# mct10/Speech-Vecalign

Measured on AMD Instinct MI355X. Metric: aligned doc-pairs/sec, higher is better.
Workload: dtype bf16; 1 GPU; synthetic 4096x4096 d=1024 bf16 embeddings, 4 overlap layers/side, 10 alignment types, band 14, coarse-to-fine (max_size_full_dp=300), 1024 doc-pairs per GPU per step; pipeline=1, N=4096, M=4096, d=1024, overlaps=4, parallelism=dp1 (pairs sharded, no collective)

## Files before the change

include/svx.h:

```cpp
#ifndef SVX_H
#define SVX_H

#include <stdint.h>

#ifdef __cplusplus
extern "C" {
#endif

typedef struct svx_ctx svx_ctx;

enum svx_dtype { SVX_F32 = 0, SVX_F16 = 1, SVX_BF16 = 2 };

enum svx_status {
    SVX_OK = 0,
    SVX_ERR_ARG = 1,
    SVX_ERR_OVERLAPS = 2,
    SVX_ERR_HIP = 3,
    SVX_ERR_TRACEBACK = 4,
    SVX_ERR_NOMEM = 5,
    SVX_ERR_EXTEND = 6,
    SVX_ERR_PATH = 7,
    SVX_ERR_BP = 8
};

// ... 150 lines not shown

typedef struct svx_level_view {
    int32_t size0, size1, k0, k1;
    int32_t n_types, band;
    int32_t path_len, n_align;
    const float *n0, *n1;
    const double *del_penalty;
    const int32_t *searchpath;
    const float *a_b_costs;
    const int32_t *b_offset;
    const double *a_b_csum;
    const uint8_t *a_b_bp;
    const int32_t *a_b_xp, *a_b_yp;
    const int32_t *new_b_offset;
    const int32_t *alignments;
    const double *alignment_scores;
    const float *costs_1to1;
    const int32_t *x_y_tb_diag;
    const float *v0_l0, *v1_l0;
    const float *knob_scores;
    int32_t n_knob, reserved;
} svx_level_view;
int svx_debug_level(svx_ctx *ctx, int pair, int level, svx_level_view *out);
int svx_copy_to_host(svx_ctx *ctx, void *dst_host, const void *src_device, int64_t bytes);

int svx_set_profiling(svx_ctx *ctx, int on);
int svx_set_pipeline(svx_ctx *ctx, int on);
int svx_flush(svx_ctx *ctx);
double svx_stage_ms(svx_ctx *ctx, const char *stage);
int svx_stage_launches(svx_ctx *ctx, const char *stage);

#ifdef __cplusplus
}
#endif
#endif
```

speech-vecalign_amd/csrc/svx_api.hip:

```cpp
#include <stdarg.h>
#include <stdio.h>
#include <stdlib.h>
#include <string.h>

#include <chrono>
#include <functional>
#include <memory>
#include <type_traits>
#include <vector>

#include "svx_common.h"

static char g_err[512] = "";

int svx_fail(svx_ctx* ctx, int code, const char* fmt, ...) {
    char* dst = ctx ? ctx->err : g_err;
    va_list ap;
    va_start(ap, fmt);
    vsnprintf(dst, 512, fmt, ap);
    va_end(ap);
    return code;
}

static const char* kStageNames[] = {"pyr0",       "pyrN",     "pyr_aux",      "knob_scoresN", "knob",      "dense_costs",
// ... 9 lines not shown
struct StageRec {
    int stage;
    hipEvent_t a, b;
};

struct BatchParams {
    SvxTypes tfinal, t11;
    int W, B, dtype, d, nsamp, n_types;
    double frac;
    bool straight, tiles, packable;
};

struct HalfState {
    char* arena = nullptr;
    size_t arena_bytes = 0;
    SvxPairDev* pinned = nullptr;
    size_t pinned_cap = 0;
    std::vector<SvxPairDev> host;
    SvxPairDev* dpairs = nullptr;
    int n_pairs = 0;
    int maxL = 0, max_ksum = 0, max_kn = 0, max_ds0 = 0, max_ds1 = 0, max_n0 = 0, max_tnd = 0;
    int max_nblk[SVX_MAX_LEVELS] = {0}, max_A[SVX_MAX_LEVELS] = {0};
    bool any_L0 = false;
    size_t o_tickets = 0;
    size_t o_planes = 0, b_planes = 0;
    double b_pyr[SVX_MAX_LEVELS] = {0}, b_bc[SVX_MAX_LEVELS] = {0}, b_knobN = 0, b_knob0 = 0, dense_cells = 0;
    BatchParams bp;
    bool chain_pending = false;
    bool chain_done_valid = false;
    hipEvent_t front_done = nullptr, chain_done = nullptr, upload_done = nullptr;
    bool upload_valid = false;
};

struct svx_ctx_ext : svx_ctx {
    double ms[S_COUNT];
    int launches[S_COUNT];
    std::vector<StageRec> recs;
    std::vector<StageRec> pending;
    double acc_ms[S_COUNT];
    long long acc_launches[S_COUNT];
    int pipeline;
    HalfState half[2];
    int last_split;
    hipStream_t chain;
    bool chain_ready;
    std::vector<hipEvent_t> ev_pool;
    size_t ev_next;
    hipStream_t side;
    hipStream_t helper;
    hipEvent_t side_fork, side_join;
    bool side_ready;
    int last_ntypes, last_band;
};

static inline svx_ctx_ext* X(svx_ctx* c) { return static_cast<svx_ctx_ext*>(c); }

struct StageScope {
    svx_ctx_ext* c;
    StageRec r;
    bool on;
    StageScope(svx_ctx* ctx, int stage) : c(X(ctx)), on(ctx->profiling != 0) {
        r.stage = stage;
        if (on) {
            (void)hipEventCreate(&r.a);
            (void)hipEventCreate(&r.b);
            (void)hipEventRecord(r.a, c->stream);
        }
    }
    ~StageScope() {
        if (on) {
            (void)hipEventRecord(r.b, c->stream);
            c->recs.push_back(r);
        }
        c->launches[r.stage]++;
    }
// ... 18 lines not shown
    e = hipSetDevice(device_id);
    if (e != hipSuccess) return svx_fail(nullptr, SVX_ERR_HIP, "hipSetDevice: %s", hipGetErrorString(e));
    svx_ctx_ext* c = new svx_ctx_ext();
    c->device = device_id;
    c->stream = nullptr;
    c->arena = nullptr;
    c->arena_bytes = 0;
    c->arena_used = 0;
    c->err[0] = 0;
    c->profiling = 0;
    c->rows_buf = nullptr;
    c->rows_bytes = 0;
    c->rows_turn = 0;
    for (int i = 0; i < 2; i++) { c->rows_pin[i] = nullptr; c->rows_pin_cap[i] = 0; c->rows_up[i] = nullptr; c->rows_up_valid[i] = 0; }
    for (int i = 0; i < S_COUNT; i++) { c->ms[i] = -1.0; c->launches[i] = 0; }
    c->pipeline = 0;
    c->last_split = 0;
    c->chain = nullptr;
    c->chain_ready = false;
    c->ev_next = 0;
    c->last_ntypes = 0;
    c->last_band = 0;
    c->side_ready = false;
    *out = c;
    return SVX_OK;
}

int svx_destroy(svx_ctx* ctx) {
    if (!ctx) return SVX_OK;
    svx_ctx_ext* c = X(ctx);
    (void)hipSetDevice(ctx->device);
    (void)svx_flush(ctx);
    (void)hipStreamSynchronize(ctx->stream);
    if (c->chain_ready) (void)hipStreamSynchronize(c->chain);
    if (ctx->arena) (void)hipFree(ctx->arena);
    svxl_alignrows_release(ctx);
    drop_pending(c);
    for (auto& r : c->recs) { (void)hipEventDestroy(r.a); (void)hipEventDestroy(r.b); }
    if (c->side_ready) {
        (void)hipStreamSynchronize(c->side);
        (void)hipStreamDestroy(c->side);
        (void)hipStreamSynchronize(c->helper);
        (void)hipStreamDestroy(c->helper);
        (void)hipEventDestroy(c->side_fork);
        (void)hipEventDestroy(c->side_join);
    }
// ... 23 lines not shown
    if (rc) return rc;
    SVX_HIP(ctx, hipStreamSynchronize(ctx->stream));
    return SVX_OK;
}

const char* svx_last_error(const svx_ctx* ctx) { return ctx ? ctx->err : g_err; }

int64_t svx_scratch_bytes(const svx_ctx* ctx) {
    if (!ctx) return 0;
    const svx_ctx_ext* c = static_cast<const svx_ctx_ext*>(ctx);
    return (int64_t)(ctx->arena_bytes + c->half[0].arena_bytes + c->half[1].arena_bytes + ctx->rows_bytes);
}

int svx_set_pipeline(svx_ctx* ctx, int on) {
    if (!ctx || on < 0 || on > 1) return SVX_ERR_ARG;
    if (X(ctx)->pipeline != on) {
        int rc = svx_flush(ctx);
        if (rc) return rc;
    }
    X(ctx)->pipeline = on;
    return SVX_OK;
}

static void fold_pending(svx_ctx_ext* c) {
    if (c->pending.empty()) return;
    (void)svx_flush(c);
    (void)hipStreamSynchronize(c->stream);
    if (c->side_ready) { (void)hipStreamSynchronize(c->side); (void)hipStreamSynchronize(c->helper); }
    for (auto& r : c->pending) {
        float ms = 0.f;
        if (hipEventElapsedTime(&ms, r.a, r.b) == hipSuccess) { c->acc_ms[r.stage] += ms; }
        (void)hipEventDestroy(r.a);
        (void)hipEventDestroy(r.b);
    }
    c->pending.clear();
}

int svx_set_profiling(svx_ctx* ctx, int on) {
    if (!ctx) return SVX_ERR_ARG;
    svx_ctx_ext* c = X(ctx);
    drop_pending(c);
    ctx->profiling = on;
    if (on == 2)
        for (int i = 0; i < S_COUNT; i++) { c->acc_ms[i] = 0.0; c->acc_launches[i] = 0; }
    return SVX_OK;
}
// ... 243 lines not shown
    SVX_HIP(ctx, hipStreamSynchronize(ctx->stream));
    return SVX_OK;
}

extern "C" int svx_debug_level(svx_ctx* ctx, int pair, int level, svx_level_view* out) {
    NEED(ctx, ctx && out, "svx_debug_level: null argument");
    svx_ctx_ext* cx = X(ctx);
    const int total = cx->half[0].n_pairs + (cx->last_split > 0 ? cx->half[1].n_pairs : 0);
    NEED(ctx, pair >= 0 && pair < total, "svx_debug_level: pair %d of the last batch (%d pairs)", pair, total);
    const bool second = cx->last_split > 0 && pair >= cx->last_split;
    const SvxPairDev& P = second ? cx->half[1].host[pair - cx->last_split] : cx->half[0].host[pair];
    NEED(ctx, level >= 0 && level <= P.L, "svx_debug_level: level %d (the pair has %d)", level, P.L + 1);
    const SvxLevel& Lv = P.lev[level];
    memset(out, 0, sizeof(*out));
    out->size0 = Lv.n[0]; out->size1 = Lv.n[1];
    out->k0 = P.K[0]; out->k1 = P.K[1];
    out->n_types = level == 0 ? cx->last_ntypes : 1;
    out->band = cx->last_band;
    out->n0 = Lv.nrm[0]; out->n1 = Lv.nrm[1];
    out->del_penalty = Lv.pen;
    SVX_HIP(ctx, hipSetDevice(ctx->device));
    int rc = svx_synchronize(ctx);
    if (rc) return rc;
    if (Lv.n_align) SVX_HIP(ctx, hipMemcpy(&out->n_align, Lv.n_align, sizeof(int), hipMemcpyDeviceToHost));
    out->alignments = Lv.align;
    const bool refined = (level < P.L) || (P.L == 0);
    if (refined) {
        SVX_HIP(ctx, hipMemcpy(&out->path_len, Lv.path_len, sizeof(int), hipMemcpyDeviceToHost));
        out->searchpath = Lv.path;
        out->a_b_costs = Lv.costs;
        out->b_offset = Lv.boff;
        out->a_b_csum = Lv.csum;
        out->a_b_bp = Lv.bpk;
        out->a_b_xp = Lv.xp;
        out->a_b_yp = Lv.yp;
        out->new_b_offset = Lv.boff_out;
        out->alignment_scores = Lv.scores;
    }
    if (level == P.L && !P.straight) {
        out->costs_1to1 = P.dcost;
        out->x_y_tb_diag = P.dbp;
    }
    out->knob_scores = Lv.kscore;
    out->n_knob = Lv.kn;
    if (level >= 1) {
        out->v0_l0 = Lv.P[0];
        out->v1_l0 = Lv.P[1];
    }
    return SVX_OK;
}

static int plan_half(svx_ctx* ctx, HalfState& H, const BatchParams& bp, const svx_align_params* prm, const svx_pair* pairs, int n_pairs) {
    const int d = bp.d;
    const size_t esz = bp.dtype == SVX_F32 ? 4 : 2;
    const SvxTypes& tfinal = bp.tfinal;
    const int B = bp.B;
    const bool straight = bp.straight, tiles = bp.tiles, packable = bp.packable;
    int mx = 0, my = 0;
    for (int t = 0; t < tfinal.n; t++) { if (tfinal.x[t] > mx) mx = tfinal.x[t]; if (tfinal.y[t] > my) my = tfinal.y[t]; }
    std::vector<SvxPairDev>& host = H.host;
    host.assign(n_pairs, SvxPairDev());
    H.n_pairs = n_pairs;
    H.bp = bp;
    H.maxL = H.max_ksum = H.max_kn = H.max_ds0 = H.max_ds1 = H.max_n0 = H.max_tnd = 0;
    H.any_L0 = false;
    H.o_tickets = 0;
    H.o_planes = H.b_planes = 0;
    H.b_knobN = H.b_knob0 = H.dense_cells = 0;
    for (int l = 0; l < SVX_MAX_LEVELS; l++) { H.max_nblk[l] = H.max_A[l] = 0; H.b_pyr[l] = H.b_bc[l] = 0; }
    Bump bump;
    const size_t o_desc = bump.take((size_t)n_pairs * sizeof(SvxPairDev));
#define OFF(ptr_field, bytes) set_off(ptr_field, bump, bytes)
    for (int p = 0; p < n_pairs; p++) {
        const svx_pair& in = pairs[p];
        SvxPairDev& P = host[p];
        memset(&P, 0, sizeof(P));
        NEED(ctx, in.vecs0 && in.vecs1 && in.align && in.scores && in.info && in.knob_idx, "pair %d: null pointer", p);
        NEED(ctx, in.n >= 1 && in.m >= 1 && in.k0 >= 1 && in.k1 >= 1, "pair %d: empty document or no overlap layers", p);
        if (mx > in.k0) return svx_fail(ctx, SVX_ERR_OVERLAPS, "%d x overlaps requrested (via alignment_types), but vecs0 only has %d", mx, in.k0);
        if (my > in.k1) return svx_fail(ctx, SVX_ERR_OVERLAPS, "%d y overlaps requrested (via alignment_types), but vecs1 only has %d", my, in.k1);
        const int L = straight ? 0 : svx_num_levels(in.n, in.m, prm->max_size_full_dp);
        P.straight = straight ? 1 : 0;
        NEED(ctx, L < SVX_MAX_LEVELS, "pair %d: %d pyramid levels (max %d)", p, L + 1, SVX_MAX_LEVELS);
        P.v[0] = in.vecs0; P.v[1] = in.vecs1;
        P.K[0] = in.k0; P.K[1] = in.k1;
        P.L = L; P.d = d;
        P.norm_override[0] = in.norms0 != nullptr;
        P.norm_override[1] = in.norms1 != nullptr;
// ... 66 lines not shown
                if (packable) {
                    OFF(Lv.bpk, (size_t)(cap + 2) * B);
                } else {
                    OFF(Lv.xp, (size_t)(cap + 2) * B * sizeof(int));
                    OFF(Lv.yp, (size_t)(cap + 2) * B * sizeof(int));
                }
                OFF(Lv.boff_out, (size_t)(cap + 2) * sizeof(int));
            }
            if (l == 0) {
                Lv.align = in.align;
                Lv.scores = in.scores;
                Lv.n_align = in.info;
            } else {
                OFF(Lv.align, (size_t)rows_cap * 4 * sizeof(int));
                OFF(Lv.scores, (size_t)rows_cap * sizeof(double));
                OFF(Lv.n_align, sizeof(int));
            }
            const double krows = (double)K[0] * Lv.n[0] + (double)K[1] * Lv.n[1], rows = (double)Lv.n[0] + Lv.n[1];
            if (l == 0) {
                H.b_pyr[0] += krows * d * esz;
                H.b_bc[0] += krows * d * esz;
                H.b_knob0 += (double)kn * d * esz;
            } else {
                if (l == 1) H.b_pyr[1] += ((double)K[0] * in.n + (double)K[1] * in.m) * d * esz + rows * d * 4.0;
                else H.b_pyr[l] += (krows + rows) * d * 4.0;
                H.b_pyr[l - 1] += l >= 2 ? krows * d * 4.0 : 0.0;
                if (l < L) { H.b_bc[l] += rows * d * 4.0; H.b_knobN += (double)kn * d * 4.0; }
            }
        }
        const SvxLevel& top = P.lev[L];
        if (!straight) {
            if (top.n[0] > H.max_ds0) H.max_ds0 = top.n[0];
            if (top.n[1] > H.max_ds1) H.max_ds1 = top.n[1];
            H.dense_cells += (double)top.n[0] * top.n[1];
            OFF(P.dcost, (size_t)top.n[0] * top.n[1] * sizeof(float));
            OFF(P.ddot, (size_t)top.n[0] * top.n[1] * sizeof(float));
            OFF(P.dbp, (size_t)(top.n[0] + top.n[1] + 1) * (top.n[0] + 1) * sizeof(int));
        }
        if (tiles) {
            const long long TI = in.n / 32 + 1, TJ = in.m / 32 + 1;
            P.t_nd = (int)(TI + TJ - 1);
            long long tcap = (long long)P.t_nd * ((B + 64) / 32 + 2);
            if (tcap > TI * TJ) tcap = TI * TJ;
            NEED(ctx, tcap < (1ll << 30), "pair %d: too many tiles", p);
            P.t_cap = (int)tcap;
            OFF(P.t_lo, (size_t)P.t_nd * sizeof(int));
            OFF(P.t_cnt, (size_t)P.t_nd * sizeof(int));
            OFF(P.t_pref, (size_t)(P.t_nd + 1) * sizeof(int));
            OFF(P.t_flag, (size_t)P.t_cap * sizeof(int));
        }
    }
#undef OFF
    for (int p = 0; p < n_pairs; p++)
        if (host[p].t_nd > H.max_tnd) H.max_tnd = host[p].t_nd;
    if (tiles) {
        H.o_tickets = bump.take(((size_t)(H.max_tnd + 2) * n_pairs + 2) * sizeof(int));
        H.b_planes = svxl_band_tiles_scratch(tfinal);
        if (H.b_planes) H.o_planes = bump.take(H.b_planes);
    }
    if (bump.off > H.arena_bytes) {
        SVX_HIP(ctx, hipDeviceSynchronize());
        if (H.arena) SVX_HIP(ctx, hipFree(H.arena));
        H.arena = nullptr;
        H.arena_bytes = 0;
        const size_t want = bump.off + bump.off / 16 + (1 << 20);
        hipError_t e = hipMalloc(&H.arena, want);
        if (e != hipSuccess) return svx_fail(ctx, SVX_ERR_NOMEM, "scratch arena: hipMalloc(%zu) failed: %s", want, hipGetErrorString(e));
        H.arena_bytes = want;
    }
    const size_t desc_bytes = (size_t)n_pairs * sizeof(SvxPairDev);
    if (desc_bytes > H.pinned_cap) {
        SVX_HIP(ctx, hipDeviceSynchronize());
        if (H.pinned) SVX_HIP(ctx, hipHostFree(H.pinned));
        H.pinned = nullptr;
        H.pinned_cap = 0;
// ... 80 lines not shown
        return SVX_OK;
    }});
    auto sort_op = [=]() -> int {
        hipStream_t main_stream = ctx->stream;
        static const bool inline_sort = getenv("SVX_SORT_INLINE") != nullptr;
        if (parts > 1 && !inline_sort) SVX_HIP(ctx, hipStreamWaitEvent(cx->side, evs->pass[0][parts - 1], 0));
        ctx->stream = inline_sort ? main_stream : cx->side;
        int rc;
        {
            StageScope sc(ctx, S_KNOB_SORT);
            rc = svxl_knob_scores(ctx, h->dpairs, np, h->maxL, h->max_kn, h->max_n0, dtype, d, 0);
        }
        ctx->stream = main_stream;
        if (rc) return rc;
        SVX_HIP(ctx, hipEventRecord(cx->side_join, inline_sort ? main_stream : cx->side));
        return SVX_OK;
    };
    if (parts == 1) ops.push_back({0.0, -1, sort_op});
    for (int l = 0; l <= H.maxL; l++) {
        for (int q = 0; q < parts; q++) {
            const int lo = (int)((long long)np * q / parts), hi = (int)((long long)np * (q + 1) / parts);
            const double aux_us = (l == 0 ? 700.0 * waves : 250.0) / parts;
            if (parts == 1) {
                ops.push_back({aux_us, S_PYR_AUX, [=]() { return svxl_pyramid_level(ctx, h->dpairs, np, l, dtype, d, h->max_nblk[l], h->max_ksum, 0); }});
                ops.push_back({H.b_pyr[l] / (l == 0 ? 4.9e6 : 5.3e6), l == 0 ? S_PYR0 : (l == 1 ? S_PYR1 : S_PYRN),
                               [=]() { return svxl_pyramid_level(ctx, h->dpairs, np, l, dtype, d, h->max_nblk[l], h->max_ksum, 1); }});
                continue;
            }
            ops.push_back({H.b_pyr[l] / (l == 0 ? 4.9e6 : 5.3e6) / parts, l == 0 ? S_PYR0 : (l == 1 ? S_PYR1 : S_PYRN), [=]() -> int {
                hipStream_t main_stream = ctx->stream;
                int rc;
                if (l == 0 && q == 0) {
                    StageScope sc(ctx, S_PYR_AUX);
                    if ((rc = svxl_pyramid_level(ctx, h->dpairs + lo, hi - lo, l, dtype, d, h->max_nblk[l], h->max_ksum, 0))) return rc;
                } else {
                    if (l > 0) SVX_HIP(ctx, hipStreamWaitEvent(cx->helper, evs->pass[l - 1][q], 0));
                    ctx->stream = cx->helper;
                    {
                        StageScope sc(ctx, S_PYR_AUX);
                        rc = svxl_pyramid_level(ctx, h->dpairs + lo, hi - lo, l, dtype, d, h->max_nblk[l], h->max_ksum, 0);
                    }
                    ctx->stream = main_stream;
                    if (rc) return rc;
                    hipEvent_t aux_done;
                    if ((rc = next_event(ctx, &aux_done))) return rc;
                    SVX_HIP(ctx, hipEventRecord(aux_done, cx->helper));
                    SVX_HIP(ctx, hipStreamWaitEvent(main_stream, aux_done, 0));
                }
                if ((rc = svxl_pyramid_level(ctx, h->dpairs + lo, hi - lo, l, dtype, d, h->max_nblk[l], h->max_ksum, 1))) return rc;
                if ((rc = next_event(ctx, &evs->pass[l][q]))) return rc;
                SVX_HIP(ctx, hipEventRecord(evs->pass[l][q], main_stream));
                return SVX_OK;
            }});
        }
        if (parts > 1 && l == 0) ops.push_back({0.0, -1, sort_op});
    }
    if (!bp.straight) {
        ops.push_back({H.dense_cells * 2.7e-5, S_DENSE_COSTS, [=]() -> int {
            int rc = svxl_dense_costs_batch(ctx, h->dpairs, np, h->max_ds0, h->max_ds1, dtype, d);
            if (rc) return rc;
            return svxl_knob_from_dots(ctx, h->dpairs, np, h->max_kn);
        }});
    }
    if (H.maxL >= 1) {
        ops.push_back({H.b_knobN / 16.5e6, S_KNOB_SCORES, [=]() -> int {
            SVX_HIP(ctx, hipStreamWaitEvent(ctx->stream, cx->side_join, 0));
            return svxl_knob_scores(ctx, h->dpairs, np, h->maxL, h->max_kn, h->max_n0, dtype, d, 1);
        }});
    }
    ops.push_back({H.b_knob0 / 8.5e6, S_KNOB_SCORES0, [=]() -> int {
        SVX_HIP(ctx, hipStreamWaitEvent(ctx->stream, cx->side_join, 0));
        return svxl_knob_scores(ctx, h->dpairs, np, h->maxL, h->max_kn, h->max_n0, dtype, d, 2);
// ... 252 lines not shown
```

speech-vecalign_amd/csrc/svx_common.h:

```cpp
#pragma once
#include <hip/hip_runtime.h>
#include <stdint.h>
#include <stddef.h>
#include "../../include/svx.h"

#define SVX_WAVE 64

#ifndef SVX_PYR_SLOTS
#define SVX_PYR_SLOTS 32
#endif
#define SVX_BC_TA 32
#define SVX_BC_TAMAX 64
#define SVX_BC_TB 16
#define SVX_BC_ROWS 48

struct ElemF32 {
    using storage = float;
    static constexpr int VEC = 4;
    static constexpr int DT = SVX_F32;
};
struct ElemF16 {
    using storage = uint16_t;
    static constexpr int VEC = 8;
    static constexpr int DT = SVX_F16;
};
struct ElemBF16 {
    using storage = uint16_t;
    static constexpr int VEC = 8;
    static constexpr int DT = SVX_BF16;
};

__device__ __forceinline__ float bf16_to_f32(uint16_t h) { return __uint_as_float(((uint32_t)h) << 16); }
__device__ __forceinline__ float f16_to_f32(uint16_t h) { return (float)__builtin_bit_cast(_Float16, h); }
// ... 199 lines not shown
};

int svx_fail(svx_ctx* ctx, int code, const char* fmt, ...);
#define SVX_HIP(ctx, call)                                                                     \
    do {                                                                                       \
        hipError_t e_ = (call);                                                                \
        if (e_ != hipSuccess) return svx_fail(ctx, SVX_ERR_HIP, "%s: %s", #call, hipGetErrorString(e_)); \
    } while (0)
#define SVX_LAUNCH_CHECK(ctx, name)                                                            \
    do {                                                                                       \
        hipError_t e_ = hipGetLastError();                                                     \
        if (e_ != hipSuccess) return svx_fail(ctx, SVX_ERR_HIP, "launch %s: %s", name, hipGetErrorString(e_)); \
    } while (0)

void svxl_alignrows_release(svx_ctx*);
int svxl_make_norm1(svx_ctx*, float* vecs, int64_t rows, int d);
int svxl_pairsum(svx_ctx*, const float* vecs, int k, int n, int d, float* half, float* part, int nblk);
int svxl_colmean_plain(svx_ctx*, const float* part, int k, int nblk, int d, int count, float* mean);
int svxl_sub_mean(svx_ctx*, float* half, int k, int h, int d, const float* mean);
int svxl_sample_mean_plain(svx_ctx*, const float* vecs, int k, int n, int d, const int* idx, int S, float* rbar);
int svxl_norms_from_rbar(svx_ctx*, const float* vecs, int64_t rows, int d, const float* rbar, float* norms);
int svxl_gather_rows(svx_ctx*, const void* table, long long n_rows, int row_bytes, int dtype, const int* idx, long long n_out, void* out);
int svxl_pyramid_level(svx_ctx*, const SvxPairDev* pairs, int n_pairs, int level, int dtype, int d, int max_nblk,
                       int max_ksum, int part);
int svxl_score_path(svx_ctx*, const int* xx, const int* yy, int64_t n, const float* n1, const float* n2,
                    const float* v1, int rows1, const float* v2, int rows2, int d, float* out);
int svxl_knob_scores(svx_ctx*, const SvxPairDev* pairs, int n_pairs, int max_levels, int max_kn, int max_n0, int dtype, int d,
                     int part);
int svxl_dense_costs(svx_ctx*, const float* v0, int s0, const float* v1, int s1, int d, const float* n0,
                     const float* n1, int mul0, int mul1, float* costs);
int svxl_dense_costs_batch(svx_ctx*, const SvxPairDev* pairs, int n_pairs, int max_s0, int max_s1, int dtype, int d);
int svxl_knob_from_dots(svx_ctx*, const SvxPairDev* pairs, int n_pairs, int max_kn);
int svxl_band_costs(svx_ctx*, const void* v0, int k0, int n, const void* v1, int k1, int m, int d, int dtype,
                    const float* inv0, const float* inv1, const float* nrm0, const float* nrm1, const int* path,
                    int A, const SvxTypes& types, int W, float* costs, int* boff, int* status);
int svxl_band_costs_batch(svx_ctx*, const SvxPairDev* pairs, int n_pairs, int depth, int max_A, const SvxTypes& types,
                          int W, int dtype, int d);
bool svxl_band2_limits(const SvxTypes& types, int W, int depth, int dtype, int d, int* lim, int* tamax);
int svxl_band_costs2_batch(svx_ctx*, const SvxPairDev* pairs, int n_pairs, int depth, int max_A, const SvxTypes& types, int W,
                           int dtype, int d);
int svxl_band_tiles_shape(const SvxTypes& types);
size_t svxl_band_tiles_scratch(const SvxTypes& types);
int svxl_band_tiles_batch(svx_ctx*, const SvxPairDev* pairs, int n_pairs, const SvxTypes& types, int W, int dtype, int max_nd,
                          int* gpref, int* ticket, float* planes);
int svxl_dense_dp(svx_ctx*, const float* cost, int s0, int s1, float pen, double* csum, int* bp);
int svxl_dense_stage_batch(svx_ctx*, const SvxPairDev* pairs, int n_pairs, int max_s0);
int svxl_dense_traceback(svx_ctx*, const int* bp, int s0, int s1, int* align, int* count);
// ... 13 lines not shown
```

speech-vecalign_amd/csrc/svx_rows.hip:

```cpp
#include "svx_common.h"

namespace {

template <typename E, int NCH>
struct Row {
    static constexpr int VEC = E::VEC;
    static constexpr int EPL = NCH * VEC;
    using S = typename E::storage;

    __device__ static __forceinline__ void load(const S* row, int d, int lane, float* x) {
#pragma unroll
        for (int c = 0; c < NCH; c++) {
            int col = (c * SVX_WAVE + lane) * VEC;
            if (col < d) {
                gload_piece<E>(row + col, x + c * VEC);
            } else {
#pragma unroll
                for (int i = 0; i < VEC; i++) x[c * VEC + i] = 0.f;
            }
        }
    }
    __device__ static __forceinline__ void loadf(const float* v, int d, int lane, float* x) {
#pragma unroll
        for (int c = 0; c < NCH; c++) {
// ... 59 lines not shown

template <typename R, bool FULL, bool NT>
__device__ __forceinline__ void store_row_via_lds(float* dst, int d, int lane, const float* x, float* wbuf) {
    constexpr int NCH = R::EPL / R::VEC;
    static_assert(R::VEC == 8, "16-bit column map");
#pragma unroll
    for (int c = 0; c < NCH; c++) {
        float4* w4 = reinterpret_cast<float4*>(wbuf + 512 * c + 8 * lane);
        w4[0] = make_float4(x[8 * c + 0], x[8 * c + 1], x[8 * c + 2], x[8 * c + 3]);
        w4[1] = make_float4(x[8 * c + 4], x[8 * c + 5], x[8 * c + 6], x[8 * c + 7]);
    }
#pragma unroll
    for (int g = 0; g < 2 * NCH; g++) {
        const int col = 256 * g + 4 * lane;
        const float4 v = *reinterpret_cast<const float4*>(wbuf + col);
        if (FULL || col < d) {
            if (NT) gstf4_nt(dst + col, v.x, v.y, v.z, v.w);
            else gstf4(dst + col, v.x, v.y, v.z, v.w);
        }
    }
}

#define SVX_PYR_LDS_FLOATS(NCH, VEC) (6 * (NCH) * (VEC) * SVX_WAVE + 4)

template <typename R, bool FULL>
__device__ __forceinline__ void part_epilogue(float* red, int* arrive, const float* cs, float* part_out, int d, int lane, int w) {
    constexpr int EPL = R::EPL;
#pragma unroll
    for (int e = 0; e < EPL; e++) red[(w * EPL + e) * SVX_WAVE + lane] = cs[e];
    int ticket = 0;
    if (lane == 0) ticket = __hip_atomic_fetch_add(arrive, 1, __ATOMIC_ACQ_REL, __HIP_MEMORY_SCOPE_WORKGROUP);
    ticket = __builtin_amdgcn_readfirstlane(ticket);
    if (ticket != 3) return;
    float sum[EPL];
#pragma unroll
    for (int e = 0; e < EPL; e++) {
        float t = red[(0 * EPL + e) * SVX_WAVE + lane];
        t += red[(1 * EPL + e) * SVX_WAVE + lane];
        t += red[(2 * EPL + e) * SVX_WAVE + lane];
        t += red[(3 * EPL + e) * SVX_WAVE + lane];
        sum[e] = t;
    }
    R::template storef<FULL>(part_out, d, lane, sum);
}

template <typename E, int NCH, bool PAIR>
// ... 69 lines not shown
        rb_l[at] = (rbar && c < d) ? gld(rbar + c) : 0.f;
    }
    __syncthreads();
    auto lane_major = [&](const float* tab, float* out) {
#pragma unroll
        for (int g4 = 0; g4 < EPL / 4; g4++) {
            const float4 t = *reinterpret_cast<const float4*>(tab + (g4 * SVX_WAVE + lane) * 4);
            out[4 * g4 + 0] = t.x; out[4 * g4 + 1] = t.y; out[4 * g4 + 2] = t.z; out[4 * g4 + 3] = t.w;
        }
    };
    float cs[EPL];
#pragma unroll
    for (int e = 0; e < EPL; e++) cs[e] = 0.f;
    const int slot0 = blk * SVX_PYR_SLOTS + w * (SVX_PYR_SLOTS / 4);
    const int r0 = 2 * slot0;
    int r1 = r0 + 2 * (SVX_PYR_SLOTS / 4);
    r1 = r1 < n ? r1 : n;
    float xs[EPL];
    float keep_inv = 0.f, keep_nrm = 0.f;
    RawRow<E, NCH, PAIR> ring[DEPTH];
    constexpr int RPWV = 2 * (SVX_PYR_SLOTS / 4);
    static_assert(RPWV % DEPTH == 0, "whole ring revolutions");
    const int rl = r1 - 1;
    constexpr bool HOIST = EPL <= 16;
    float mu[EPL], rbv[EPL];
    if (HOIST) {
        lane_major(mu_l, mu);
        lane_major(rb_l, rbv);
    }
    if (r0 < r1) {
#pragma unroll
        for (int s = 0; s < DEPTH; s++) fetch_raw<E, NCH, PAIR, NT, FULL>(rows, inv0, (r0 + s) < rl ? (r0 + s) : rl, d, lane, ring[s]);
#pragma unroll
        for (int i = 0; i < RPWV; i++) {
            const int r = r0 + i, s = i % DEPTH;
            const int jp = r >> 1, half = i & 1;
            float x[EPL];
            decode_raw<E, NCH, PAIR>(ring[s], x);
            if (i + DEPTH < RPWV) fetch_raw<E, NCH, PAIR, NT, FULL>(rows, inv0, (r + DEPTH) < rl ? (r + DEPTH) : rl, d, lane, ring[s]);
            if (r >= r1) continue;
            if (mean) {
                if (!HOIST) lane_major(mu_l, mu);
#pragma unroll
                for (int e = 0; e < EPL; e++) x[e] = x[e] - mu[e];
            }
            float ss = 0.f;
// ... 7 lines not shown
            if (rbar) {
                if (!HOIST) lane_major(rb_l, rbv);
                float dt = 0.f;
#pragma unroll
                for (int e = 0; e < EPL; e++) dt += x[e] * rbv[e];
                dt = wave_sum(dt);
                keep_nrm = lane == i ? 1.0f - dt : keep_nrm;
            }
            keep_inv = lane == i ? rden : keep_inv;
            if (vn_out) {
                if constexpr (E::VEC == 8) store_row_via_lds<R, FULL, false>(vn_out + (size_t)r * d, d, lane, x, red + w * EPL * SVX_WAVE);
                else R::template storef<FULL>(vn_out + (size_t)r * d, d, lane, x);
            }
            if (next || part_out) {
                if (half == 0) {
#pragma unroll
                    for (int e = 0; e < EPL; e++) xs[e] = x[e];
                } else {
#pragma unroll
                    for (int e = 0; e < EPL; e++) {
                        xs[e] = xs[e] + x[e];
                        cs[e] += xs[e];
                    }
                    if (next) {
                        if constexpr (E::VEC == 8) store_row_via_lds<R, FULL, true>(next + (size_t)jp * d, d, lane, xs, red + w * EPL * SVX_WAVE);
                        else R::template storef_nt<FULL>(next + (size_t)jp * d, d, lane, xs);
                    }
                }
            }
        }
    }
    if (lane < RPWV && r0 + lane < r1) {
        if (inv_out) gst(inv_out + r0 + lane, keep_inv);
        if (nrm_out && rbar) gst(nrm_out + r0 + lane, keep_nrm);
    }
    if (part_out) part_epilogue<R, FULL>(red, arrive, cs, part_out, d, lane, w);
}

template <typename E, int NCH, bool FULL = false>
__device__ void pyr0_block(const typename E::storage* rows, int n, int d, const float* rbar, float* inv_out, float* nrm_out,
                           float* part_out, int blk, float* lds) {
    using R = Row<E, NCH>;
    constexpr int EPL = R::EPL;
    constexpr int DP = EPL * SVX_WAVE;
    constexpr int DEPTH = E::VEC == 8 ? 4 : 2;
    const int lane = threadIdx.x & 63, w = threadIdx.x >> 6;
    float* rb_l = lds;
// ... 132 lines not shown
    }
#pragma unroll
    for (int e = 0; e < EPL; e++) lds[(w * EPL + e) * SVX_WAVE + lane] = acc[e];
    __syncthreads();
    for (int i2 = threadIdx.x; i2 < EPL * SVX_WAVE; i2 += blockDim.x) {
        const int e = i2 / SVX_WAVE, l = i2 % SVX_WAVE;
        const int col = R::col_of(e, l);
        if (col < d) {
            float s = lds[(0 * EPL + e) * SVX_WAVE + l];
            s += lds[(1 * EPL + e) * SVX_WAVE + l];
            s += lds[(2 * EPL + e) * SVX_WAVE + l];
            s += lds[(3 * EPL + e) * SVX_WAVE + l];
            rbar[col] = s / (float)total;
        }
    }
}

#ifndef SVX_PYR_MINW
#define SVX_PYR_BOUNDS __launch_bounds__(256)
#else
#define SVX_PYR_BOUNDS __launch_bounds__(256, SVX_PYR_MINW)
#endif
template <typename E, int NCH, int MODE, bool FULL>
__global__ SVX_PYR_BOUNDS void k_pyramid(const SvxPairDev* __restrict__ pairs, int level) {
    constexpr bool LV0 = MODE == 1;
    __shared__ float lds[SVX_PYR_LDS_FLOATS(NCH, E::VEC)];
    const SvxPairDev& P = pairs[blockIdx.z];
    if (level > P.L) return;
    int side, k;
    if ((int)blockIdx.y < P.K[0]) {
        side = 0;
        k = blockIdx.y;
    } else {
        side = 1;
        k = blockIdx.y - P.K[0];
        if (k >= P.K[1]) return;
    }
    const SvxLevel& Lv = P.lev[level];
    if ((int)blockIdx.x >= Lv.nblk[side]) return;
    const int n = Lv.n[side], d = P.d;
    using S = typename E::storage;
    const int n0 = P.lev[0].n[side];
    const S* rows = LV0 ? reinterpret_cast<const S*>(P.v[side]) + (size_t)k * n * d
                        : (MODE == 2 ? reinterpret_cast<const S*>(P.v[side]) + (size_t)k * n0 * d
                                     : reinterpret_cast<const S*>(Lv.P[side] + (size_t)k * n * d));
    const float* inv0 = MODE == 2 ? P.lev[0].inv[side] + (size_t)k * n0 : nullptr;
    const float* mean = LV0 ? nullptr : Lv.mean[side] + (size_t)k * d;
    const bool want_nrm = !(LV0 && P.norm_override[side]);
    const float* rbar = want_nrm ? Lv.rbar[1 - side] : nullptr;
    float* inv_out = LV0 ? Lv.inv[side] + (size_t)k * n : nullptr;
    float* nrm_out = want_nrm ? Lv.nrm[side] + (size_t)k * n : nullptr;
    float* vn_out = (!LV0 && k == 0) ? Lv.P[side] : nullptr;
    const bool has_next = level < P.L;
    float* next = (has_next && !LV0) ? P.lev[level + 1].P[side] + (size_t)k * (n / 2) * d : nullptr;
    float* part = has_next ? P.lev[level + 1].part[side] + ((size_t)k * Lv.nblk[side] + blockIdx.x) * d : nullptr;
#ifndef SVX_PYR_NT
#define SVX_PYR_NT 0
#endif
    constexpr bool NT = ((SVX_PYR_NT >> (MODE == 1 ? 0 : (MODE == 2 ? 1 : 2))) & 1) != 0;
#ifndef SVX_PYR0_GENERIC
    if constexpr (LV0) {
        pyr0_block<E, NCH, FULL>(rows, n, d, rbar, inv_out, nrm_out, part, blockIdx.x, lds);
        return;
    }
#endif
    pyr_block<E, NCH, MODE == 2, NT, FULL>(rows, n, d, mean, rbar, inv_out, nrm_out, vn_out, next, part, blockIdx.x, lds, inv0);
}

__global__ __launch_bounds__(256) void k_colmean(const SvxPairDev* __restrict__ pairs, int level) {
    const SvxPairDev& P = pairs[blockIdx.z];
    if (level > P.L || level < 1) return;
    int side, k;
    if ((int)blockIdx.y < P.K[0]) {
        side = 0;
        k = blockIdx.y;
    } else {
        side = 1;
        k = blockIdx.y - P.K[0];
// ... 239 lines not shown
    return SVX_OK;
}

int svxl_sample_mean_plain(svx_ctx* ctx, const float* vecs, int k, int n, int d, const int* idx, int S, float* rbar) {
#define M(N) hipLaunchKernelGGL(k_sample_mean_plain<N>, dim3(1), dim3(256), 0, ctx->stream, vecs, k, n, d, idx, S, rbar)
    SVX_SWITCH_NCH_F32(d, M)
#undef M
    SVX_LAUNCH_CHECK(ctx, "k_sample_mean_plain");
    return SVX_OK;
}

int svxl_norms_from_rbar(svx_ctx* ctx, const float* vecs, int64_t rows, int d, const float* rbar, float* norms) {
    if (rows <= 0) return SVX_OK;
    int64_t nb = (rows + 3) / 4;
    if (nb > 8192) nb = 8192;
#define M(N) hipLaunchKernelGGL(k_rownorms_plain<N>, dim3((unsigned)nb), dim3(256), 0, ctx->stream, vecs, rows, d, rbar, norms)
    SVX_SWITCH_NCH_F32(d, M)
#undef M
    SVX_LAUNCH_CHECK(ctx, "k_rownorms_plain");
    return SVX_OK;
}

int svxl_pyramid_level(svx_ctx* ctx, const SvxPairDev* pairs, int n_pairs, int level, int dtype, int d, int max_nblk,
                       int max_ksum, int part) {
    if (n_pairs <= 0 || max_nblk <= 0) return SVX_OK;
    hipStream_t st = ctx->stream;
    if (part == 0 && level >= 1) {
        hipLaunchKernelGGL(k_colmean, dim3((d + 255) / 256, max_ksum, n_pairs), dim3(256), 0, st, pairs, level);
        SVX_LAUNCH_CHECK(ctx, "k_colmean");
    }
#define LAUNCH(E, N, MODE)                                                                                             \
    do {                                                                                                               \
        if (part == 0) hipLaunchKernelGGL((k_sample_mean<E, N, MODE>), dim3(2, n_pairs), dim3(256), 0, st, pairs, level); \
        else if (d == N * E::VEC * SVX_WAVE) hipLaunchKernelGGL((k_pyramid<E, N, MODE, true>), dim3(max_nblk, max_ksum, n_pairs), dim3(256), 0, st, pairs, level); \
        else hipLaunchKernelGGL((k_pyramid<E, N, MODE, false>), dim3(max_nblk, max_ksum, n_pairs), dim3(256), 0, st, pairs, level); \
    } while (0)
    const int mode = level == 0 ? 1 : (level == 1 ? 2 : 0);
    if (mode == 0) {
#define M(N) LAUNCH(ElemF32, N, 0)
        SVX_SWITCH_NCH_F32(d, M)
#undef M
    } else if (dtype == SVX_F32) {
#define M(N) do { if (mode == 1) LAUNCH(ElemF32, N, 1); else LAUNCH(ElemF32, N, 2); } while (0)
        SVX_SWITCH_NCH_F32(d, M)
#undef M
    } else if (dtype == SVX_F16) {
#define M(N) do { if (mode == 1) LAUNCH(ElemF16, N, 1); else LAUNCH(ElemF16, N, 2); } while (0)
        SVX_SWITCH_NCH_16(d, M)
#undef M
    } else {
#define M(N) do { if (mode == 1) LAUNCH(ElemBF16, N, 1); else LAUNCH(ElemBF16, N, 2); } while (0)
        SVX_SWITCH_NCH_16(d, M)
#undef M
    }
#undef LAUNCH
    SVX_LAUNCH_CHECK(ctx, "k_pyramid");
    return SVX_OK;
}
// ... 27 lines not shown
```

speech-vecalign_amd/svx/_lib.py:

```python
import ctypes
import os
import threading

_HERE = os.path.dirname(os.path.abspath(__file__))
LIB_PATH = os.environ.get("SVX_LIB") or os.path.join(_HERE, "libsvx.so")

SVX_F32, SVX_F16, SVX_BF16 = 0, 1, 2
SVX_MAX_TYPES = 128
SVX_MAX_LEVELS = 16
SVX_MARGIN_RATIO, SVX_MARGIN_DISTANCE, SVX_MARGIN_ABSOLUTE = 0, 1, 2
SVX_SEARCH_COARSE_TO_FINE, SVX_SEARCH_STRAIGHT = 0, 1

SVX_OK, SVX_ERR_ARG, SVX_ERR_OVERLAPS, SVX_ERR_HIP, SVX_ERR_TRACEBACK = 0, 1, 2, 3, 4
SVX_ERR_NOMEM, SVX_ERR_EXTEND, SVX_ERR_PATH, SVX_ERR_BP = 5, 6, 7, 8

DEVICE_ERRORS = {
    SVX_ERR_TRACEBACK: "traceback bug",
    SVX_ERR_BP: "got unknown value",
    SVX_ERR_EXTEND: "asked to extend alignments but already bigger than requested",
    SVX_ERR_PATH: "search path is not a unit-step lattice path",
}

c_int, c_i64, c_f32, c_f64, c_vp = ctypes.c_int, ctypes.c_int64, ctypes.c_float, ctypes.c_double, ctypes.c_void_p

# ... 82 lines not shown
    "svx_knn_search_groups": (c_int, [c_vp, c_vp, c_int, c_vp, c_int, c_int, c_int, c_vp, c_vp, c_int, c_vp, c_vp]),
    "svx_margin_scores": (c_int, [c_vp, c_vp, c_vp, c_int, c_i64, c_int, c_vp, c_vp, c_int, c_vp]),
    "svx_knn_list_means": (c_int, [c_vp, c_vp, c_i64, c_int, c_vp]),
    "svx_margin_candidates": (c_int, [c_vp, c_vp, c_vp, c_i64, c_int, c_vp, c_vp, c_i64, c_i64, c_int, c_vp, c_vp, c_vp]),
    "svx_mine_greedy": (c_i64, [c_vp, c_i64, c_vp, c_vp, c_i64, c_i64, c_vp]),
    "svx_mt19937_choice": (c_int, [c_vp, ctypes.POINTER(ctypes.c_int32), c_i64, c_i64, c_vp]),
    "svx_norm_index_count": (c_i64, [c_int, c_int, c_int, c_int, c_int, c_int, c_int, c_int]),
    "svx_knob_index_count": (c_i64, [c_int, c_int, c_int, c_int]),
    "svx_draw_indices": (c_int, [c_vp, ctypes.POINTER(ctypes.c_int32), c_int, c_int, c_int, c_int, c_int, c_int, c_int, c_int, c_int,
                                 c_vp, c_vp]),
    "svx_candidate_table": (c_int, [ctypes.c_char_p, ctypes.c_char_p, ctypes.c_char_p, c_int, c_vp, c_int,
                                    ctypes.POINTER(ctypes.c_int32), ctypes.POINTER(c_i64), ctypes.c_char_p, c_int]),
    "svx_format_alignments": (c_i64, [c_vp, c_vp, c_i64, c_vp, c_i64]),
    "svx_num_levels": (c_int, [c_int, c_int, c_int]),
    "svx_knob_count": (c_i64, [c_int, c_int, c_int]),
    "svx_align_batch": (c_int, [c_vp, ctypes.POINTER(AlignParams), ctypes.POINTER(Pair), c_int]),
    "svx_alignment_rows": (c_int, [c_vp, c_int, c_int, ctypes.POINTER(Pair), c_int, c_f64, c_i64, c_vp, c_vp, c_vp, c_vp, c_int, c_vp, c_vp]),
    "svx_concat_rows": (c_int, [c_vp, c_int, c_int, ctypes.POINTER(Pair), ctypes.POINTER(Frames), c_int, ctypes.POINTER(ConcatParams), c_i64,
                                c_vp, c_vp, c_vp, c_vp, c_int, c_vp, c_vp]),
    "svx_debug_level": (c_int, [c_vp, c_int, c_int, ctypes.POINTER(LevelView)]),
    "svx_copy_to_host": (c_int, [c_vp, c_vp, c_vp, c_i64]),
    "svx_set_profiling": (c_int, [c_vp, c_int]),
    "svx_set_pipeline": (c_int, [c_vp, c_int]),
    "svx_flush": (c_int, [c_vp]),
    "svx_stage_ms": (c_f64, [c_vp, ctypes.c_char_p]),
    "svx_stage_launches": (c_int, [c_vp, ctypes.c_char_p]),
}

EXPORTS = tuple(_SIGS)

_lib = None
_lock = threading.Lock()


def load():
    global _lib
    with _lock:
        if _lib is None:
            if not os.path.exists(LIB_PATH):
                raise ImportError(
                    "libsvx.so not found at %s: build it with `make -C speech-vecalign_amd/csrc` "
                    "(there is no CPU fallback)" % LIB_PATH)
            L = ctypes.CDLL(LIB_PATH)
            for name, (res, args) in _SIGS.items():
                fn = getattr(L, name)
                fn.restype = res
# ... 28 lines not shown
        if os.environ.get("SVX_PIPELINE") == "1":
            self.set_pipeline(True)

    def use_current_stream(self):
        self.lib.svx_set_stream(self.h, c_vp(self.torch.cuda.current_stream(self.tdev).cuda_stream))

    def check(self, rc):
        if rc != 0:
            msg = self.lib.svx_last_error(self.h).decode()
            if rc == SVX_ERR_OVERLAPS:
                raise Exception(msg)
            raise SvxError(rc, msg)

    def sync(self):
        self.check(self.lib.svx_synchronize(self.h))
        del self._held[:]

    def set_pipeline(self, on):
        if self._held:
            self.flush()
        self.check(self.lib.svx_set_pipeline(self.h, 1 if on else 0))
        self.pipeline = bool(on)

    def flush(self):
        self.check(self.lib.svx_flush(self.h))
        del self._held[:]

    def hold(self, batch):
        if self.pipeline and not any(b is batch for b in self._held):
            if len(self._held) >= 4:
                self.flush()
            self._held.append(batch)

    def __del__(self):
        try:
            if getattr(self, "h", None):
                self.lib.svx_destroy(self.h)
                self.h = None
        except Exception:
            pass


_ctxs = {}


def context(device=None):
# ... 12 lines not shown
```

Baseline: 9703 doc-pairs/s.

## Build lean pyramid by skipping unused upper overlap layers and unsampled rows

Adds a lean pyramid mode, on by default, that skips building coarse-level pyramid planes for overlap layers k>=1 at the top level. When the next level is only used by the sampler, it writes just the rows the sampler indexes, using a per-block skip bitmask built with wave ballots. The skipped work is rebuilt on demand in the debug path, and an env var or API call restores the full stack. This cuts memory writes and bandwidth in the pyramid stage, at the cost of more kernel branching and a risk of stale data if any consumer reads the skipped planes.

```diff
diff --git a/include/svx.h b/include/svx.h
--- a/include/svx.h
+++ b/include/svx.h
@@ -196,6 +196,7 @@
     int32_t n_knob, reserved;
 } svx_level_view;
 int svx_debug_level(svx_ctx *ctx, int pair, int level, svx_level_view *out);
+int svx_set_full_stack(svx_ctx *ctx, int on);
 int svx_copy_to_host(svx_ctx *ctx, void *dst_host, const void *src_device, int64_t bytes);
 
 int svx_set_profiling(svx_ctx *ctx, int on);
diff --git a/speech-vecalign_amd/csrc/svx_api.hip b/speech-vecalign_amd/csrc/svx_api.hip
--- a/speech-vecalign_amd/csrc/svx_api.hip
+++ b/speech-vecalign_amd/csrc/svx_api.hip
@@ -55,6 +55,8 @@
     int maxL = 0, max_ksum = 0, max_kn = 0, max_ds0 = 0, max_ds1 = 0, max_n0 = 0, max_tnd = 0;
     int max_nblk[SVX_MAX_LEVELS] = {0}, max_A[SVX_MAX_LEVELS] = {0};
     bool any_L0 = false;
+    int pyr_what = SVX_PYR_FULL;
+    bool stack_lean = false;
     size_t o_tickets = 0;
     size_t o_planes = 0, b_planes = 0;
     double b_pyr[SVX_MAX_LEVELS] = {0}, b_bc[SVX_MAX_LEVELS] = {0}, b_knobN = 0, b_knob0 = 0, dense_cells = 0;
@@ -84,6 +86,7 @@
     hipEvent_t side_fork, side_join;
     bool side_ready;
     int last_ntypes, last_band;
+    int full_stack;
 };
 
 static inline svx_ctx_ext* X(svx_ctx* c) { return static_cast<svx_ctx_ext*>(c); }
@@ -148,6 +151,10 @@
     c->last_ntypes = 0;
     c->last_band = 0;
     c->side_ready = false;
+    {
+        const char* e = getenv("SVX_PYR_LEAN");
+        c->full_stack = (e && atoi(e) == 0) ? 1 : 0;
+    }
     *out = c;
     return SVX_OK;
 }
@@ -217,6 +224,12 @@
     return SVX_OK;
 }
 
+int svx_set_full_stack(svx_ctx* ctx, int on) {
+    if (!ctx || on < 0 || on > 1) return SVX_ERR_ARG;
+    X(ctx)->full_stack = on;
+    return SVX_OK;
+}
+
 static void fold_pending(svx_ctx_ext* c) {
     if (c->pending.empty()) return;
     (void)svx_flush(c);
@@ -506,6 +519,14 @@
     SVX_HIP(ctx, hipSetDevice(ctx->device));
     int rc = svx_synchronize(ctx);
     if (rc) return rc;
+    for (int h = 0; h < (cx->last_split > 0 ? 2 : 1); h++) {
+        HalfState& H = cx->half[h];
+        if (!H.stack_lean) continue;
+        for (int l = 1; l <= H.maxL; l++)
+            if ((rc = svxl_pyramid_level(ctx, H.dpairs, H.n_pairs, l, H.bp.dtype, H.bp.d, H.max_nblk[l], H.max_ksum, 1, SVX_PYR_REST))) return rc;
+        SVX_HIP(ctx, hipStreamSynchronize(ctx->stream));
+        H.stack_lean = false;
+    }
     if (Lv.n_align) SVX_HIP(ctx, hipMemcpy(&out->n_align, Lv.n_align, sizeof(int), hipMemcpyDeviceToHost));
     out->alignments = Lv.align;
     const bool refined = (level < P.L) || (P.L == 0);
@@ -548,6 +569,9 @@
     H.bp = bp;
     H.maxL = H.max_ksum = H.max_kn = H.max_ds0 = H.max_ds1 = H.max_n0 = H.max_tnd = 0;
     H.any_L0 = false;
+    H.pyr_what = X(ctx)->full_stack ? SVX_PYR_FULL : SVX_PYR_LEAN;
+    H.stack_lean = false;
+    const bool lean = H.pyr_what == SVX_PYR_LEAN;
     H.o_tickets = 0;
     H.o_planes = H.b_planes = 0;
     H.b_knobN = H.b_knob0 = H.dense_cells = 0;
@@ -660,9 +684,10 @@
                 H.b_bc[0] += krows * d * esz;
                 H.b_knob0 += (double)kn * d * esz;
             } else {
-                if (l == 1) H.b_pyr[1] += ((double)K[0] * in.n + (double)K[1] * in.m) * d * esz + rows * d * 4.0;
-                else H.b_pyr[l] += (krows + rows) * d * 4.0;
-                H.b_pyr[l - 1] += l >= 2 ? krows * d * 4.0 : 0.0;
+                const bool only0 = lean && l == L;
+                if (l == 1) H.b_pyr[1] += (only0 ? (double)in.n + in.m : (double)K[0] * in.n + (double)K[1] * in.m) * d * esz + rows * d * 4.0;
+                else H.b_pyr[l] += ((only0 ? rows : krows) + rows) * d * 4.0;
+                H.b_pyr[l - 1] += l >= 2 ? (only0 ? rows : krows) * d * 4.0 : 0.0;
                 if (l < L) { H.b_bc[l] += rows * d * 4.0; H.b_knobN += (double)kn * d * 4.0; }
             }
         }
@@ -689,6 +714,7 @@
         }
     }
 #undef OFF
+    H.stack_lean = lean && H.maxL >= 1;
     for (int p = 0; p < n_pairs; p++)
         if (host[p].t_nd > H.max_tnd) H.max_tnd = host[p].t_nd;
     if (tiles) {
@@ -815,9 +841,9 @@
             const int lo = (int)((long long)np * q / parts), hi = (int)((long long)np * (q + 1) / parts);
             const double aux_us = (l == 0 ? 700.0 * waves : 250.0) / parts;
             if (parts == 1) {
-                ops.push_back({aux_us, S_PYR_AUX, [=]() { return svxl_pyramid_level(ctx, h->dpairs, np, l, dtype, d, h->max_nblk[l], h->max_ksum, 0); }});
+                ops.push_back({aux_us, S_PYR_AUX, [=]() { return svxl_pyramid_level(ctx, h->dpairs, np, l, dtype, d, h->max_nblk[l], h->max_ksum, 0, h->pyr_what); }});
                 ops.push_back({H.b_pyr[l] / (l == 0 ? 4.9e6 : 5.3e6), l == 0 ? S_PYR0 : (l == 1 ? S_PYR1 : S_PYRN),
-                               [=]() { return svxl_pyramid_level(ctx, h->dpairs, np, l, dtype, d, h->max_nblk[l], h->max_ksum, 1); }});
+                               [=]() { return svxl_pyramid_level(ctx, h->dpairs, np, l, dtype, d, h->max_nblk[l], h->max_ksum, 1, h->pyr_what); }});
                 continue;
             }
             ops.push_back({H.b_pyr[l] / (l == 0 ? 4.9e6 : 5.3e6) / parts, l == 0 ? S_PYR0 : (l == 1 ? S_PYR1 : S_PYRN), [=]() -> int {
@@ -825,13 +851,13 @@
                 int rc;
                 if (l == 0 && q == 0) {
                     StageScope sc(ctx, S_PYR_AUX);
-                    if ((rc = svxl_pyramid_level(ctx, h->dpairs + lo, hi - lo, l, dtype, d, h->max_nblk[l], h->max_ksum, 0))) return rc;
+                    if ((rc = svxl_pyramid_level(ctx, h->dpairs + lo, hi - lo, l, dtype, d, h->max_nblk[l], h->max_ksum, 0, h->pyr_what))) return rc;
                 } else {
                     if (l > 0) SVX_HIP(ctx, hipStreamWaitEvent(cx->helper, evs->pass[l - 1][q], 0));
                     ctx->stream = cx->helper;
                     {
                         StageScope sc(ctx, S_PYR_AUX);
-                        rc = svxl_pyramid_level(ctx, h->dpairs + lo, hi - lo, l, dtype, d, h->max_nblk[l], h->max_ksum, 0);
+                        rc = svxl_pyramid_level(ctx, h->dpairs + lo, hi - lo, l, dtype, d, h->max_nblk[l], h->max_ksum, 0, h->pyr_what);
                     }
                     ctx->stream = main_stream;
                     if (rc) return rc;
@@ -840,7 +866,7 @@
                     SVX_HIP(ctx, hipEventRecord(aux_done, cx->helper));
                     SVX_HIP(ctx, hipStreamWaitEvent(main_stream, aux_done, 0));
                 }
-                if ((rc = svxl_pyramid_level(ctx, h->dpairs + lo, hi - lo, l, dtype, d, h->max_nblk[l], h->max_ksum, 1))) return rc;
+                if ((rc = svxl_pyramid_level(ctx, h->dpairs + lo, hi - lo, l, dtype, d, h->max_nblk[l], h->max_ksum, 1, h->pyr_what))) return rc;
                 if ((rc = next_event(ctx, &evs->pass[l][q]))) return rc;
                 SVX_HIP(ctx, hipEventRecord(evs->pass[l][q], main_stream));
                 return SVX_OK;
diff --git a/speech-vecalign_amd/csrc/svx_common.h b/speech-vecalign_amd/csrc/svx_common.h
--- a/speech-vecalign_amd/csrc/svx_common.h
+++ b/speech-vecalign_amd/csrc/svx_common.h
@@ -9,6 +9,9 @@
 #ifndef SVX_PYR_SLOTS
 #define SVX_PYR_SLOTS 32
 #endif
+#define SVX_PYR_FULL 0
+#define SVX_PYR_LEAN 1
+#define SVX_PYR_REST 2
 #define SVX_BC_TA 32
 #define SVX_BC_TAMAX 64
 #define SVX_BC_TB 16
@@ -254,7 +257,7 @@
 int svxl_norms_from_rbar(svx_ctx*, const float* vecs, int64_t rows, int d, const float* rbar, float* norms);
 int svxl_gather_rows(svx_ctx*, const void* table, long long n_rows, int row_bytes, int dtype, const int* idx, long long n_out, void* out);
 int svxl_pyramid_level(svx_ctx*, const SvxPairDev* pairs, int n_pairs, int level, int dtype, int d, int max_nblk,
-                       int max_ksum, int part);
+                       int max_ksum, int part, int what);
 int svxl_score_path(svx_ctx*, const int* xx, const int* yy, int64_t n, const float* n1, const float* n2,
                     const float* v1, int rows1, const float* v2, int rows2, int d, float* out);
 int svxl_knob_scores(svx_ctx*, const SvxPairDev* pairs, int n_pairs, int max_levels, int max_kn, int max_n0, int dtype, int d,
diff --git a/speech-vecalign_amd/csrc/svx_rows.hip b/speech-vecalign_amd/csrc/svx_rows.hip
--- a/speech-vecalign_amd/csrc/svx_rows.hip
+++ b/speech-vecalign_amd/csrc/svx_rows.hip
@@ -105,6 +105,8 @@
 }
 
 #define SVX_PYR_LDS_FLOATS(NCH, VEC) (6 * (NCH) * (VEC) * SVX_WAVE + 4)
+#define SVX_PYR_LDS_SKIP(DP) (6 * (DP) + 1)
+static_assert(SVX_PYR_SLOTS == 32, "one bit of the skip word per slot");
 
 template <typename R, bool FULL>
 __device__ __forceinline__ void part_epilogue(float* red, int* arrive, const float* cs, float* part_out, int d, int lane, int w) {
@@ -220,6 +222,7 @@
     constexpr int RPWV = 2 * (SVX_PYR_SLOTS / 4);
     static_assert(RPWV % DEPTH == 0, "whole ring revolutions");
     const int rl = r1 - 1;
+    const unsigned skip = next ? __builtin_amdgcn_readfirstlane(reinterpret_cast<const unsigned*>(lds)[SVX_PYR_LDS_SKIP(DP)] >> (w * (RPWV / 2))) : 0u;
     constexpr bool HOIST = EPL <= 16;
     float mu[EPL], rbv[EPL];
     if (HOIST) {
@@ -273,7 +276,7 @@
                         xs[e] = xs[e] + x[e];
                         cs[e] += xs[e];
                     }
-                    if (next) {
+                    if (next && !((skip >> (i >> 1)) & 1u)) {
                         if constexpr (E::VEC == 8) store_row_via_lds<R, FULL, true>(next + (size_t)jp * d, d, lane, xs, red + w * EPL * SVX_WAVE);
                         else R::template storef_nt<FULL>(next + (size_t)jp * d, d, lane, xs);
                     }
@@ -452,7 +455,7 @@
 #define SVX_PYR_BOUNDS __launch_bounds__(256, SVX_PYR_MINW)
 #endif
 template <typename E, int NCH, int MODE, bool FULL>
-__global__ SVX_PYR_BOUNDS void k_pyramid(const SvxPairDev* __restrict__ pairs, int level) {
+__global__ SVX_PYR_BOUNDS void k_pyramid(const SvxPairDev* __restrict__ pairs, int level, int what) {
     constexpr bool LV0 = MODE == 1;
     __shared__ float lds[SVX_PYR_LDS_FLOATS(NCH, E::VEC)];
     const SvxPairDev& P = pairs[blockIdx.z];
@@ -466,6 +469,8 @@
         k = blockIdx.y - P.K[0];
         if (k >= P.K[1]) return;
     }
+    const bool upper = !LV0 && k >= 1;
+    if (what == SVX_PYR_REST ? !upper : (what == SVX_PYR_LEAN && upper && level == P.L)) return;
     const SvxLevel& Lv = P.lev[level];
     if ((int)blockIdx.x >= Lv.nblk[side]) return;
     const int n = Lv.n[side], d = P.d;
@@ -476,14 +481,33 @@
                                      : reinterpret_cast<const S*>(Lv.P[side] + (size_t)k * n * d));
     const float* inv0 = MODE == 2 ? P.lev[0].inv[side] + (size_t)k * n0 : nullptr;
     const float* mean = LV0 ? nullptr : Lv.mean[side] + (size_t)k * d;
-    const bool want_nrm = !(LV0 && P.norm_override[side]);
+    const bool sampler_only = upper && level + 1 == P.L;
+    const bool want_nrm = !(LV0 && P.norm_override[side]) && !(upper && what == SVX_PYR_LEAN);
     const float* rbar = want_nrm ? Lv.rbar[1 - side] : nullptr;
     float* inv_out = LV0 ? Lv.inv[side] + (size_t)k * n : nullptr;
     float* nrm_out = want_nrm ? Lv.nrm[side] + (size_t)k * n : nullptr;
     float* vn_out = (!LV0 && k == 0) ? Lv.P[side] : nullptr;
     const bool has_next = level < P.L;
-    float* next = (has_next && !LV0) ? P.lev[level + 1].P[side] + (size_t)k * (n / 2) * d : nullptr;
-    float* part = has_next ? P.lev[level + 1].part[side] + ((size_t)k * Lv.nblk[side] + blockIdx.x) * d : nullptr;
+    bool want_next = has_next && !LV0;
+    if (what == SVX_PYR_REST) want_next = sampler_only;
+    if (!LV0 && threadIdx.x < SVX_WAVE) {
+        unsigned skip = 0u;
+        const SvxLevel& Up = P.lev[has_next ? level + 1 : level];
+        const int S_up = Up.S[side];
+        if (what == SVX_PYR_LEAN && sampler_only && S_up <= SVX_WAVE) {
+            int kr = -1;
+            if ((int)threadIdx.x < S_up && Up.sidx[side] != nullptr) {
+                kr = gld(Up.sidx[side] + (size_t)k * S_up + threadIdx.x);
+                kr = kr < 0 ? 0 : (kr >= n / 2 ? n / 2 - 1 : kr);
+            }
+            const int slot0 = blockIdx.x * SVX_PYR_SLOTS;
+#pragma unroll
+            for (int j = 0; j < SVX_PYR_SLOTS; j++) skip |= (__ballot(kr == slot0 + j) != 0ull ? 0u : 1u) << j;
+        }
+        if (threadIdx.x == 0) reinterpret_cast<unsigned*>(lds)[SVX_PYR_LDS_SKIP(NCH * E::VEC * SVX_WAVE)] = skip;
+    }
+    float* next = want_next ? P.lev[level + 1].P[side] + (size_t)k * (n / 2) * d : nullptr;
+    float* part = (has_next && what != SVX_PYR_REST) ? P.lev[level + 1].part[side] + ((size_t)k * Lv.nblk[side] + blockIdx.x) * d : nullptr;
 #ifndef SVX_PYR_NT
 #define SVX_PYR_NT 0
 #endif
@@ -769,8 +793,9 @@
 }
 
 int svxl_pyramid_level(svx_ctx* ctx, const SvxPairDev* pairs, int n_pairs, int level, int dtype, int d, int max_nblk,
-                       int max_ksum, int part) {
+                       int max_ksum, int part, int what) {
     if (n_pairs <= 0 || max_nblk <= 0) return SVX_OK;
+    if (what == SVX_PYR_REST && (part == 0 || level < 1)) return SVX_OK;
     hipStream_t st = ctx->stream;
     if (part == 0 && level >= 1) {
         hipLaunchKernelGGL(k_colmean, dim3((d + 255) / 256, max_ksum, n_pairs), dim3(256), 0, st, pairs, level);
@@ -779,8 +804,8 @@
 #define LAUNCH(E, N, MODE)                                                                                             \
     do {                                                                                                               \
         if (part == 0) hipLaunchKernelGGL((k_sample_mean<E, N, MODE>), dim3(2, n_pairs), dim3(256), 0, st, pairs, level); \
-        else if (d == N * E::VEC * SVX_WAVE) hipLaunchKernelGGL((k_pyramid<E, N, MODE, true>), dim3(max_nblk, max_ksum, n_pairs), dim3(256), 0, st, pairs, level); \
-        else hipLaunchKernelGGL((k_pyramid<E, N, MODE, false>), dim3(max_nblk, max_ksum, n_pairs), dim3(256), 0, st, pairs, level); \
+        else if (d == N * E::VEC * SVX_WAVE) hipLaunchKernelGGL((k_pyramid<E, N, MODE, true>), dim3(max_nblk, max_ksum, n_pairs), dim3(256), 0, st, pairs, level, what); \
+        else hipLaunchKernelGGL((k_pyramid<E, N, MODE, false>), dim3(max_nblk, max_ksum, n_pairs), dim3(256), 0, st, pairs, level, what); \
     } while (0)
     const int mode = level == 0 ? 1 : (level == 1 ? 2 : 0);
     if (mode == 0) {
diff --git a/speech-vecalign_amd/svx/_lib.py b/speech-vecalign_amd/svx/_lib.py
--- a/speech-vecalign_amd/svx/_lib.py
+++ b/speech-vecalign_amd/svx/_lib.py
@@ -128,6 +128,7 @@
     "svx_copy_to_host": (c_int, [c_vp, c_vp, c_vp, c_i64]),
     "svx_set_profiling": (c_int, [c_vp, c_int]),
     "svx_set_pipeline": (c_int, [c_vp, c_int]),
+    "svx_set_full_stack": (c_int, [c_vp, c_int]),
     "svx_flush": (c_int, [c_vp]),
     "svx_stage_ms": (c_f64, [c_vp, ctypes.c_char_p]),
     "svx_stage_launches": (c_int, [c_vp, ctypes.c_char_p]),
@@ -202,6 +203,9 @@
         self.check(self.lib.svx_set_pipeline(self.h, 1 if on else 0))
         self.pipeline = bool(on)
 
+    def set_full_stack(self, on):
+        self.check(self.lib.svx_set_full_stack(self.h, 1 if on else 0))
+
     def flush(self):
         self.check(self.lib.svx_flush(self.h))
         del self._held[:]
```

Result: no change. 9791 doc-pairs/s (median of 3 runs) (+0.9%).
